# bigpon/QPNet

Measured on AMD Instinct MI355X. Metric: train steps/sec (batch-1 chunk-steps of RF+20000 samples, aggregate over GPUs), higher is better.
Workload: dtype f32; 1 GPU; config[1]: paper-size SI-QPNet (C=64,S=256,4F+4A) training step, forward+CE+backward+Adam on one chunk of 20900 samples (RF 946 + batch_length 19954), batch 1 per GPU; global_batch=1, parallelism=dp1 (utterance-sharded chunks, one flat-gradient all-reduce per step), backend=none, world_size=1, aux_1x1=frame rate (hoisted: K = 128 + one 4-deep step)

## Files before the change

### qpnet_amd/csrc/train_bwd.hip

```cpp
#include "train_common.h"
#include "train_post.h"
#include "qpn_handle.h"
#include <string.h>
#include <stdlib.h>
#include <math.h>

template <int MT>
__global__ __launch_bounds__(512) void k_post_bwd(TrainParams p, TrainBwd bw) {
    constexpr int TM = 16 * MT;
    extern __shared__ float sm[];
    const int S = p.S, Q = p.Q, LC = p.LC;
    const int ldp = tr_lda(Q > S ? Q : S), ldr = tr_lda(S);
    float* P = sm; float* R = sm + TM * ldp;
    const int b = blockIdx.y, t0 = blockIdx.x * TM;
    const int tid = threadIdx.x, lane = tid & 63, wave = tid >> 6;
    const int NTS = S / 16;
    const int npairs = (NTS + 1) / 2;
    const int np0 = wave < npairs ? wave : 0;
    const int pnt[2] = {2 * np0, (2 * np0 + 1 < NTS) ? 2 * np0 + 1 : 2 * np0};
    float my[2][MT][4], ms[2][MT][4];
    auto mask_load = [&](const float* src, float (&m)[2][MT][4]) {
#pragma unroll
        for (int j = 0; j < 2; ++j)
#pragma unroll
            for (int mt = 0; mt < MT; ++mt)
#pragma unroll
                for (int i = 0; i < 4; ++i) {
                    const int r = t0 + 16 * mt + 4 * (lane >> 4) + i;
                    m[j][mt][i] = src[((size_t)b * p.BL + r) * S + 16 * pnt[j] + (lane & 15)];
                }
    };
#define PIN8(m) asm volatile("" :: "v"(m[0][0][0]), "v"(m[0][0][1]), "v"(m[0][0][2]), "v"(m[0][0][3]), "v"(m[1][0][0]), "v"(m[1][0][1]), "v"(m[1][0][2]), "v"(m[1][0][3]))
    mask_load(p.Y0, my);
    for (int idx = tid; idx < TM * (Q / 2); idx += 512) {
        const int r = idx / (Q / 2), k = (idx - r * (Q / 2)) * 2;
        float2 v = make_float2(0.f, 0.f);
        if (t0 + r < p.BL) v = *(const float2*)(bw.dlogits + ((size_t)b * p.BL + t0 + r) * Q + k);
        *(float2*)(P + (size_t)r * ldp + k) = v;
    }
    __syncthreads();
    mask_load(p.S0, ms);
    PIN8(my);
    if (MT > 1) {
#pragma unroll
        for (int mt = 1; mt < MT; ++mt) asm volatile("" :: "v"(my[0][mt][0]), "v"(my[0][mt][1]), "v"(my[0][mt][2]), "v"(my[0][mt][3]), "v"(my[1][mt][0]), "v"(my[1][mt][1]), "v"(my[1][mt][2]), "v"(my[1][mt][3]));
    }
    for (int pb = 0; pb < npairs; pb += 8) {
        const int np = pb + wave;
        if (np < npairs) {
            const int nt0 = 2 * np, nt1 = (2 * np + 1 < NTS) ? 2 * np + 1 : 2 * np;
            f32x4 acc[MT][2];
#pragma unroll
            for (int mt = 0; mt < MT; ++mt) { acc[mt][0] = (f32x4){0, 0, 0, 0}; acc[mt][1] = (f32x4){0, 0, 0, 0}; }
            const int nts[2] = {nt0, nt1};
            wave_gemm<MT, 2>(acc, P, ldp, p.wp + p.p2t_f4, NTS, nts, Q, lane);
#pragma unroll
            for (int j = 0; j < 2; ++j) {
                if (j && nt1 == nt0) break;
// ... 360 lines not shown
#pragma unroll
            for (int i = 0; i < 4; ++i) Os[(size_t)(4 * (lane >> 4) + i) * ldo + 16 * nt + (lane & 15)] = acc[j][i];
        }
        TR_LDS_BARRIER();
#pragma unroll
        for (int i = 0; i < 4; ++i) {
            const int r = 4 * wave + i, n = n0 + r;
            const bool in = n < N1;
            const float own = Os[(size_t)r * ldo + lane] + Dx[(size_t)r * ldx + lane];
            float* da = DAout + (__umul24((unsigned)n, (unsigned)C) + lane);
            *(in ? da : dmy + lane) = own;
            const float past = Os[(size_t)r * ldo + C + lane];
            float* db = DBout + (__umul24((unsigned)tprow[i], (unsigned)C) + lane);
            db = in ? db : dmy + 128 + lane;
            if (ly.adaptive) atomicAdd(db, past);
            else *db = past;
            if constexpr (!HOIST) if (lane < Ap) {
                float* dh = DH + (__umul24((unsigned)n, (unsigned)Ap) + lane);
                atomicAdd(in ? dh : dmy + 192 + lane, Os[(size_t)r * ldo + 2 * C + lane]);
            }
        }
        if constexpr (HOIST) {
            if (lane < 16) {
                float* dp = bw.DPA + cpoff + 16 * wave + lane;
                atomicAdd(dp, dacc[0]); atomicAdd(dp + C, dacc[1]); atomicAdd(dp + 2 * C, dacc[2]); atomicAdd(dp + 3 * C, dacc[3]);
                float* ep = bw.EB + (size_t)(l * TR_EB_SLOTS + (blockIdx.x & (TR_EB_SLOTS - 1))) * 2 * C + 16 * wave + lane;
                atomicAdd(ep, eacc[0]); atomicAdd(ep + C, eacc[1]);
            }
            if (tid < 16 && n0 + tid < N1) GWl[n0 + tid] = (Gp[tid] + Gp[16 + tid]) + (Gp[32 + tid] + Gp[48 + tid]);
        }
        store_rows(t + 1 < t_last ? t + 1 : t_last, sm + ((ti + 1) & 1) * 4 * 16 * ldx);
#pragma unroll
        for (int i = 0; i < 4; ++i) tprow[i] = tpnext[i];
        if constexpr (HOIST) {
#pragma unroll
            for (int i = 0; i < 4; ++i) { cwj[i] = nwj[i]; cpa[i] = npa[i]; }
            cpoff = npoff;
        }
    }
}

struct Wg2 {
    const float* A; const float* A2; size_t A_lstride; int lda, M;
    int rowsA;
    int bmode; const float* B1; const float* B2; size_t B_lstride; int ldb, N, Nvalid;
    int rowsB;
    const float* hup; const int* tap; int C, Ap;
    const int* xc;
    int nb, nlayers;
    float* slab; int gstage;
    int row0A[TR_MAXL], row0B[TR_MAXL], R[TR_MAXL];
    int goff[TR_MAXL], gbias[TR_MAXL], tap_off[TR_MAXL], dil[TR_MAXL];
    int ldc, ncol_groups;
};

struct Wg2L {
    const float* A; const float* A2; const float* B1; const float* B2; const float* hup; const int* tap;
    int lda, ldb, M, Ng, Nvalid, rowsA, rowsB, row0A, row0B, C, Ap, dil, nb, ncol0, rend;
    unsigned uR;
};

template <int NB>
__device__ __forceinline__ void wg_taps(const Wg2L& q, int rs, int (&tp)[NB], bool b_act, int b_row0, int b_rstep) {
#pragma unroll
    for (int k = 0; k < NB; ++k) {
        const int r = b_row0 + k * b_rstep, rr = rs + r;
        int v = 0;
        if (b_act && r < 32 && rr < q.rend) {
            const unsigned b = q.nb > 1 ? (unsigned)rr / q.uR : 0u; const int i = rr - (int)(b * q.uR);
            const int nloc = q.row0B + i;
            v = q.tap ? q.tap[(size_t)b * q.rowsB + nloc] : nloc - q.dil;
        }
        tp[k] = v;
    }
}

template <int BMODE, int NA, int NB>
__device__ __forceinline__ void wg_fetch(const Wg2L& q, int rs, float4 (&ra)[NA], float4 (&ra2)[NA], float4 (&rb)[NB], float4 (&rb2)[NB], const int (&tpv)[NB],
                                         bool a_act, int a_row0, int a_rstep, int a_col, bool b_act, int b_row0, int b_rstep, int b_col) {
#pragma unroll
    for (int k = 0; k < NA; ++k) {
        const int r = a_row0 + k * a_rstep, rr = rs + r;
        float4 v = make_float4(0.f, 0.f, 0.f, 0.f), v2 = v;
        if (a_act && r < 32 && rr < q.rend && a_col < q.M) {
            const unsigned b = q.nb > 1 ? (unsigned)rr / q.uR : 0u; const int i = rr - (int)(b * q.uR);
            const size_t o = ((size_t)b * q.rowsA + q.row0A + i) * q.lda + a_col;
            v = *(const float4*)(q.A + o);
            if (q.A2) v2 = *(const float4*)(q.A2 + o);
        }
        ra[k] = v; ra2[k] = v2;
    }
#pragma unroll
    for (int k = 0; k < NB; ++k) {
        const int r = b_row0 + k * b_rstep, rr = rs + r;
        const int n = q.ncol0 + b_col;
        float4 v = make_float4(0.f, 0.f, 0.f, 0.f), v2 = make_float4(1.f, 1.f, 1.f, 1.f);
        if (b_act && r < 32 && rr < q.rend && b_col < q.Ng && n < q.Nvalid) {
            const unsigned b = q.nb > 1 ? (unsigned)rr / q.uR : 0u; const int i = rr - (int)(b * q.uR);
            const int nloc = q.row0B + i;
            const size_t row = (size_t)b * q.rowsB + nloc;
            if (BMODE <= 1) v = *(const float4*)(q.B1 + row * q.ldb + n);
            else if (BMODE == 2) { v = *(const float4*)(q.B1 + row * q.ldb + n); v2 = *(const float4*)(q.B2 + row * q.ldb + n); }
            else {
                if (n < q.C) v = *(const float4*)(q.B1 + row * q.C + n);
                else if (n < 2 * q.C) v = *(const float4*)(q.B1 + ((size_t)b * q.rowsB + tpv[k]) * q.C + (n - q.C));
                else v = *(const float4*)(q.hup + row * q.Ap + (n - 2 * q.C));
// ... 321 lines not shown
                    else v = rb[k];
                    if (BMODE == 1) { v.x = fmaxf(v.x, 0.f); v.y = fmaxf(v.y, 0.f); v.z = fmaxf(v.z, 0.f); v.w = fmaxf(v.w, 0.f); }
                    else if (BMODE == 2) { v.x *= rb2[k].x; v.y *= rb2[k].y; v.z *= rb2[k].z; v.w *= rb2[k].w; }
                    { const bool ok = (okB >> k) & 1u; v.x = ok ? v.x : 0.f; v.y = ok ? v.y : 0.f; v.z = ok ? v.z : 0.f; v.w = ok ? v.w : 0.f; }
                    *(float4*)(Bb + (size_t)r * ldB + b_col) = v;
                }
            }
        }
    };
    auto ksteps = [&](int buf, int k0, int k1) {
        const float* Ab = As + buf * BUF; const float* Bb = Bs + buf * BUF;
#pragma unroll
        for (int ks = k0; ks < k1; ++ks) {
            float bfr[NT];
#pragma unroll
            for (int nt = 0; nt < NT; ++nt) bfr[nt] = Bb[(4 * ks + g) * ldB + 16 * nt + cl];
#pragma unroll
            for (int mi = 0; mi < MPW; ++mi) {
                const float a = Ab[(4 * ks + g) * ldA + 16 * (wave + 4 * mi) + cl];
#pragma unroll
                for (int nt = 0; nt < NT; ++nt) acc[mi][nt] = __builtin_amdgcn_mfma_f32_16x16x4f32(a, bfr[nt], acc[mi][nt], 0, 0, 0);
            }
        }
    };
    for (int rs = rbeg; rs < rend; rs += RS) {
        to_lds(0);
        __syncthreads();
        if (rs + RS < rend) {
            fetch(rs + RS);
            if (BMODE == 3 && rs + 2 * RS < rend) taps(rs + 2 * RS);
        }
        ksteps(0, 0, RS / 4);
        __syncthreads();
    }
    float* out = w.slab + (size_t)ch * w.gstage;
#pragma unroll
    for (int mi = 0; mi < MPW; ++mi) {
        const int mt = wave + 4 * mi;
#pragma unroll
        for (int nt = 0; nt < NT; ++nt) {
#pragma unroll
            for (int i = 0; i < 4; ++i) {
                const int m = 16 * mt + 4 * (lane >> 4) + i, nn = 16 * nt + (lane & 15);
                out[goff + (size_t)m * w.ldc + ncol0 + nn] = acc[mi][nt][i];
            }
        }
    }
    if (gbias >= 0) {
        *(float4*)(sm + (size_t)a_row0 * Mp + a_col) = cs4;
        __syncthreads();
        if (tid < Mp) { float s = 0.f; for (int r = 0; r < ARS; ++r) s += sm[r * Mp + tid]; out[gbias + tid] = s; }
    }
}
template <int BMODE, int MPW, int NT, bool TWO_A, int MINW = 1>
__global__ __launch_bounds__(256, MINW) void k_wgrad3(Wg2 w, int nch) {
    wgrad3_body<BMODE, MPW, NT, TWO_A>(w, nch, blockIdx.x, blockIdx.y, blockIdx.z);
}

#ifndef QPN_WGRAD_MINW
#define QPN_WGRAD_MINW 2
#endif
template <int BMODE, int MPW, int NT, bool TWO_A>
static void launch_wgrad3_k(const Wg2& w, int nch, size_t lds, hipStream_t stream) {
    constexpr int MINW = (MPW == 4 && NT == 4 && !TWO_A) ? QPN_WGRAD_MINW : 1;
    if (lds > 64 * 1024) (void)hipFuncSetAttribute((const void*)k_wgrad3<BMODE, MPW, NT, TWO_A, MINW>, hipFuncAttributeMaxDynamicSharedMemorySize, (int)lds);
    hipLaunchKernelGGL((k_wgrad3<BMODE, MPW, NT, TWO_A, MINW>), dim3(nch, w.nlayers, w.ncol_groups), dim3(256), lds, stream, w, nch);
}
template <int BMODE, int MPW, int NT>
static bool wgrad3_fits(const Wg2& w) {
    const int Ng = w.N / w.ncol_groups;
    if (w.bmode != BMODE) return false;
    if (w.rowsB >= (1 << 24) || (int64_t)w.rowsB * (w.C > w.ldb ? w.C : w.ldb) >= (1ll << 32)) return false;
    if (w.M != 64 * MPW || Ng != 16 * NT || w.N % w.ncol_groups || (w.Nvalid != w.N && (w.ncol_groups != 1 || w.Nvalid % 4))) return false;
    if (BMODE == 3 && (w.ldb != w.C || w.ncol_groups != 1 || (w.C % 4) || (w.Ap % 4) || !w.tap)) return false;
    if (BMODE == 3) for (int l = 0; l < w.nlayers; ++l) if (w.tap_off[l] < 0) return false;
    return true;
}
template <int MPW, int NT> static constexpr size_t wgrad3_lds() { return (size_t)32 * (tr_ldt(64 * MPW) + tr_ldt(16 * NT)) * sizeof(float); }
template <int BMODE, int MPW, int NT>
static bool launch_wgrad3(const Wg2& w, int nch, hipStream_t stream) {
    if (!wgrad3_fits<BMODE, MPW, NT>(w)) return false;
    const size_t lds = wgrad3_lds<MPW, NT>();
    if (w.A2) launch_wgrad3_k<BMODE, MPW, NT, true>(w, nch, lds, stream);
    else launch_wgrad3_k<BMODE, MPW, NT, false>(w, nch, lds, stream);
    return true;
}
static bool wgrad3_any(const Wg2& w, int nch, bool generic, hipStream_t stream) {
    if (w.bmode == 4) return launch_wgrad3<4, 1, 8>(w, nch, stream) || launch_wgrad3<4, 1, 4>(w, nch, stream);
    if (generic) return false;
    switch (w.bmode) {
    case 3: return launch_wgrad3<3, 2, 11>(w, nch, stream) || launch_wgrad3<3, 2, 8>(w, nch, stream) || launch_wgrad3<3, 1, 7>(w, nch, stream);
    case 0: return launch_wgrad3<0, 1, 4>(w, nch, stream) || launch_wgrad3<0, 4, 4>(w, nch, stream);
    case 1: return launch_wgrad3<1, 4, 4>(w, nch, stream);
    default: return false;
    }
}

static int wgrad_col_groups(int M, int N) {
    const int nt_max = M <= 64 ? 4 : M <= 128 ? 12 : 8;
    for (int g = 1; g <= N / 16; ++g)
        if (N % g == 0 && (N / g) % 4 == 0 && (N / g + 15) / 16 <= nt_max) return g;
    return 1;
}

static bool wgrad2_any(const Wg2& w, int nch, bool generic, hipStream_t stream) {
    if (w.M > 256 && w.bmode != 4) {
        bool ok = true;
        for (int m0 = 0; m0 < w.M && ok; m0 += 256) {
            Wg2 sub = w;
            sub.A = w.A + m0; if (w.A2) sub.A2 = w.A2 + m0;
            sub.M = w.M - m0 < 256 ? w.M - m0 : 256;
            for (int l = 0; l < w.nlayers; ++l) { sub.goff[l] = w.goff[l] + m0 * w.ldc; if (w.gbias[l] >= 0) sub.gbias[l] = w.gbias[l] + m0; }
            sub.ncol_groups = wgrad_col_groups(sub.M, sub.N);
            ok = wgrad2_any(sub, nch, generic, stream);
        }
        return ok;
    }
    if (wgrad3_any(w, nch, generic, stream)) return true;
    switch (w.bmode) {
    case 4: return false;
    case 1: return wgrad2_mode<1>(w, nch, stream);
    case 2: return wgrad2_mode<2>(w, nch, stream);
    case 3: return wgrad2_mode<3>(w, nch, stream);
    default: return wgrad2_mode<0>(w, nch, stream);
    }
}

__global__ void k_reduce_grad_s(const float* __restrict__ slab, const int* __restrict__ gdst, const int* __restrict__ gdst_list, const int* __restrict__ gzero, int n_gzero,
                                int nch, int gstage, int64_t n, float* __restrict__ g, float scale, int append_scale, int s0, int s1, int skip0, int skip1, int tail,
                                const int* __restrict__ status, int flag_again) {
    int64_t i = (int64_t)blockIdx.x * blockDim.x + threadIdx.x + s0;
    if (flag_again && append_scale && i == s0) g[n + 1] = (status && *status) ? 1.f : 0.f;
    if (i < s1) {
        if (i >= skip0 && i < skip1) return;
        const int k0 = gdst[i], k1 = gdst[i + 1];
        if (k0 == k1) return;
        float a = 0.f;
        const float* sp = slab + i;
        int c = 0;
        for (; c + 8 <= nch; c += 8) {
            float v[8];
#pragma unroll
            for (int k = 0; k < 8; ++k) v[k] = sp[(size_t)(c + k) * gstage];
            a += ((v[0] + v[1]) + (v[2] + v[3])) + ((v[4] + v[5]) + (v[6] + v[7]));
        }
        for (; c < nch; ++c) a += sp[(size_t)c * gstage];
        a *= scale;
        for (int k = k0; k < k1; ++k) g[gdst_list[k]] = a;
        return;
    }
    if (!tail) return;
    const int64_t j = i - s1;
    if (j < n_gzero) g[gzero[j]] = 0.f;
    else if (append_scale && j < n_gzero + 4 && !(flag_again && j == n_gzero + 1)) g[n + (j - n_gzero)] = j == n_gzero ? scale : (j == n_gzero + 1 && status && *status) ? 1.f : 0.f;
}

__global__ __launch_bounds__(256) void k_causal_bwd(TrainParams p, TrainBwd bw, int rows_per_wg, int CB) {
    extern __shared__ float tab[];
// ... 188 lines not shown
            if (lds_c > 48 * 1024) QPN_HIP(hipFuncSetAttribute((const void*)k_causal_bwd, hipFuncAttributeMaxDynamicSharedMemorySize, (int)lds_c));
            hipLaunchKernelGGL(k_causal_bwd, dim3(nwg), dim3(256), lds_c, stream, p, bw, rpw, CB);
        }
        if (p.U > 0 && !up_done && !p.hoist) launch_up_bwd(p, bw, stream);
        if (p.hoist && ag && !up_done) launch_aux_tail(p, bw, *ag, stream);
    }
    qpn_prof_mark(PG_GRAD_TAIL, stream);
    QPN_HIP(hipGetLastError());
    return QPN_OK;
}

bool qpn_stack_bwd_fits(const TrainParams& p);
int qpn_launch_stack_bwd(const TrainParams& p, const TrainBwd& bw, const StackQ& q, const TrainKnobs& k, hipStream_t stream);
bool qpn_stack_bwd_w_fits(const TrainParams& p);
int qpn_launch_stack_bwd_w(const TrainParams& p, const TrainBwd& bw, const StackQ& q, const TrainKnobs& k, hipStream_t stream);

void qpn_launch_post_fb(const TrainParams& p, const TrainBwd& bw, hipStream_t stream) {
    constexpr int MTW = 5;
    const size_t ldsw = (size_t)16 * MTW * (tr_lda(256) + 2 * tr_lda(64)) * sizeof(float);
    (void)hipFuncSetAttribute((const void*)k_post_fb_w<MTW>, hipFuncAttributeMaxDynamicSharedMemorySize, (int)ldsw);
    hipLaunchKernelGGL((k_post_fb_w<MTW>), dim3((p.BL + 16 * MTW - 1) / (16 * MTW), p.B), dim3(512), ldsw, stream, p, bw, 1);
}

int qpn_launch_bwd(const TrainParams& p, const TrainBwd& bw, const TrainKnobs& k, const AuxGeom& ag, const StackQ* sq, hipStream_t stream, bool post_done) {
    const int C = p.C, S = p.S, Q = p.Q, L = p.L, B = p.B, N1 = p.N1, BL = p.BL;
    const TrainSlabs& sl = *bw.sl;
    const bool off32 = N1 < (1 << 24) && (int64_t)N1 * (p.LC > 2 * C ? p.LC : 2 * C) < (1ll << 32);
    const bool persist = C == 64 && (p.Ktp == 176 || p.hoist) && p.Ap <= 64 && off32 && k.persist_bwd;
    const bool stack_q = persist && k.stack_q_bwd && sq && sq->flags && p.qctl && qpn_stack_bwd_fits(p);
    const bool wr_summed = stack_q;
    const size_t nDX = (size_t)B * N1 * C;
    const size_t lds_post = (size_t)16 * (tr_lda(Q > S ? Q : S) + tr_lda(S)) * sizeof(float);
    const size_t lds_layer = (size_t)16 * (4 * tr_lda(C) + tr_lda(2 * C)) * sizeof(float);
    if (lds_post > 160 * 1024 || lds_layer > 160 * 1024) { qpn_set_error("backward tiles do not fit LDS"); return QPN_EINVAL; }
    hipStream_t side = bw.side; hipEvent_t ev_fork = bw.ev_fork, ev_join = bw.ev_join;
    const bool overlap = side && !qpn_prof_serial() && !k.serial;
    const bool post_wide = S == 256 && Q == 256 && C == 64 && (p.LC == 256 || p.LC == 512) && k.post_wide;
    const bool zero_in_post = post_wide && k.zero_in_post;
    if (post_done) { }
    else if (!zero_in_post) qpn_launch_zero_dx(p, bw, stream);
    if (post_done) { }
    else if (post_wide) {
        constexpr int MTW = 5;
        const size_t ldsw = (size_t)16 * MTW * tr_lda(256) * sizeof(float);
        QPN_HIP(hipFuncSetAttribute((const void*)k_post_bwd_w<MTW>, hipFuncAttributeMaxDynamicSharedMemorySize, (int)ldsw));
        hipLaunchKernelGGL((k_post_bwd_w<MTW>), dim3((BL + 16 * MTW - 1) / (16 * MTW), B), dim3(512), ldsw, stream, p, bw, zero_in_post ? 1 : 0);
    } else {
        if (lds_post > 48 * 1024) (void)hipFuncSetAttribute((const void*)k_post_bwd<1>, hipFuncAttributeMaxDynamicSharedMemorySize, (int)lds_post);
        hipLaunchKernelGGL((k_post_bwd<1>), dim3((BL + 15) / 16, B), dim3(512), lds_post, stream, p, bw);
    }
    qpn_prof_mark(PG_POST_BWD, stream);
    const int nch = bw.nch;
    int nch_side_ = nch;
    const bool gen = k.wgrad_generic;
    Wg2 wbase; memset(&wbase, 0, sizeof(wbase));
    wbase.slab = bw.slab; wbase.gstage = bw.gstage; wbase.nb = B; wbase.C = C; wbase.Ap = p.Ap; wbase.hup = p.HUP; wbase.tap = p.TAP; wbase.ncol_groups = 1;
    bool ok = true;
    auto launch_skip_post = [&](hipStream_t st) {
        Wg2 w = wbase;
        {
            w.nlayers = L;
            w.A = bw.DS0; w.A2 = nullptr; w.A_lstride = 0; w.lda = S; w.M = S; w.rowsA = BL;
            w.bmode = 0; w.B1 = p.TH; w.B2 = nullptr; w.B_lstride = nDX; w.ldb = C; w.N = C; w.Nvalid = C; w.rowsB = N1; w.ldc = C;
            w.ncol_groups = wgrad_col_groups(w.M, w.N);
            for (int l = 0; l < L; ++l) { w.row0A[l] = 0; w.row0B[l] = N1 - BL; w.R[l] = BL; w.goff[l] = sl.g_ws[l]; w.gbias[l] = l == 0 ? sl.g_bs : -1; w.tap_off[l] = -1; }
            ok = ok && wgrad2_any(w, nch_side_, gen, st);
            qpn_prof_mark(PG_WGRAD_SKIP, st);
        }
        {
            w.nlayers = 1; w.A_lstride = w.B_lstride = 0; w.B2 = nullptr; w.bmode = 1; w.rowsA = w.rowsB = BL;
            w.row0A[0] = w.row0B[0] = 0; w.R[0] = BL; w.tap_off[0] = -1;
            w.ncol_groups = S % 64 == 0 ? S / 64 : 1;
            w.A = bw.dlogits; w.lda = Q; w.M = Q; w.B1 = p.Y0; w.ldb = S; w.N = S; w.Nvalid = S; w.ldc = S; w.goff[0] = sl.g_p2; w.gbias[0] = sl.g_bp2;
            if (Q == S && k.post_pair) {
                w.nlayers = 2;
                w.A_lstride = (size_t)(bw.DY0 - bw.dlogits); w.B_lstride = (size_t)(p.S0 - p.Y0);
                w.row0A[1] = w.row0B[1] = 0; w.R[1] = BL; w.tap_off[1] = -1; w.goff[1] = sl.g_p1; w.gbias[1] = sl.g_bp1;
                ok = ok && wgrad2_any(w, nch_side_, gen, st);
            } else {
                ok = ok && wgrad2_any(w, nch_side_, gen, st);
                w.A = bw.DY0; w.lda = S; w.M = S; w.B1 = p.S0; w.goff[0] = sl.g_p1; w.gbias[0] = sl.g_bp1;
                ok = ok && wgrad2_any(w, nch_side_, gen, st);
            }
            qpn_prof_mark(PG_WGRAD_POST, st);
        }
    };
    auto build_w1 = [&]() {
        Wg2 w = wbase;
        w.A = bw.DZ; w.A2 = nullptr; w.A_lstride = (size_t)B * N1 * 2 * C; w.lda = 2 * C; w.M = 2 * C; w.rowsA = N1;
        w.bmode = 3; w.B1 = p.X; w.B2 = nullptr; w.B_lstride = nDX; w.ldb = C; w.N = p.Ktp; w.Nvalid = p.hoist ? 2 * C : 2 * C + p.Ap; w.rowsB = N1;
        w.nlayers = L; w.ldc = p.Ktp; w.ncol_groups = wgrad_col_groups(w.M, w.N);
        for (int l = 0; l < L; ++l) {
            const TrLayer& ly = p.layers[l];
            w.row0A[l] = w.row0B[l] = ly.s_out; w.R[l] = N1 - ly.s_out; w.goff[l] = sl.g_w1[l]; w.gbias[l] = sl.g_b1[l];
            w.tap_off[l] = ly.tap_off; w.dil[l] = ly.dilation;
        }
        return w;
    };
    auto build_wr = [&]() {
        Wg2 w = wbase;
        w.A = bw.DXA[0] + nDX; w.A2 = wr_summed ? nullptr : bw.DXB[0] + nDX; w.A_lstride = nDX; w.lda = C; w.M = C; w.rowsA = N1;
        w.bmode = 0; w.B1 = p.TH; w.B2 = nullptr; w.B_lstride = nDX; w.ldb = C; w.N = C; w.Nvalid = C; w.rowsB = N1; w.ldc = C;
        w.nlayers = L; w.ncol_groups = wgrad_col_groups(w.M, w.N);
        for (int l = 0; l < L; ++l) {
            w.row0A[l] = w.row0B[l] = p.layers[l].s_out;
            w.R[l] = l == L - 1 ? 0 : N1 - p.layers[l].s_out; w.goff[l] = sl.g_wr[l]; w.gbias[l] = sl.g_br[l]; w.tap_off[l] = -1; w.dil[l] = 0;
        }
// ... 84 lines not shown
```

### qpnet_amd/csrc/train_common.h

```cpp
#pragma once
#include "qpn_common.h"

typedef float f32x4 __attribute__((ext_vector_type(4)));

#define TR_MAXL QPN_MAX_LAYERS

__host__ __device__ static inline int tr_lda(int K) { return ((K + 29) / 32) * 32 + 2; }
__host__ __device__ static inline int tr_ldt(int N) { return ((N + 15) / 32) * 32 + 16; }

struct TrLayer {
    int adaptive, dilation;
    int s_in, s_out;
    int tap_off;
    int w1_f4, wr_f4;
    int w1t_f4, wrt_f4;
    int bias1, biasr;
};

struct TrainParams {
    int C, S, Q, A, Ap, L, U;
    int B, T, F, Td, BL, N1, N0, maxd;
    int Kt, Ktp;
    int LC;
    const float* flat;
// ... 29 lines not shown
    TrLayer layers[TR_MAXL];
};

struct TrainSlabs {
    int g_w1[TR_MAXL], g_b1[TR_MAXL], g_wr[TR_MAXL], g_br[TR_MAXL], g_ws[TR_MAXL], g_bs;
    int g_p1, g_bp1, g_p2, g_bp2;
    int g_early0, g_early1;
    int g_cw, g_cb;
};

struct TrainBwd {
    const float* dlogits; float* gflat;
    float* DXA[2]; float* DXB[2];
    float* DZ;
    float* DS0; float* DY0;
    float* DGS;
    float* DHUP;
    float* DPA;
    float* GW;
    float* EB;
    float* slab;
    const int* gdst; const int* gdst_list;
    const int* gzero; int n_gzero;
    int nch, gstage;
    int64_t n_params;
    const struct TrainSlabs* sl;
    float gscale;
    int append_scale;
    const int* status;
    hipStream_t side; hipEvent_t ev_fork, ev_join, ev_mid;
    hipEvent_t ev_early; int* early_recorded;
};


struct AuxGeom { int auxS[TR_MAXL], auxT[TR_MAXL], bias1[TR_MAXL], s_out[TR_MAXL]; };
struct AuxArgs {
    const float* flat; const float* h; float* PA; float* bp; const float* DPA; const float* EB; const float* GW; float* gflat;
    float gscale; int C, A, L, B, F, U, N1, nfr, ffirst; int64_t up_w, up_b;
    AuxGeom g;
};
static inline AuxArgs tr_aux_args(const TrainParams& p, const TrainBwd* bw, const AuxGeom& ag) {
    AuxArgs a; a.flat = p.flat; a.h = p.h; a.PA = p.PA; a.bp = p.bp; a.DPA = bw ? bw->DPA : nullptr; a.EB = bw ? bw->EB : nullptr; a.GW = bw ? bw->GW : nullptr;
    a.gflat = bw ? bw->gflat : nullptr; a.gscale = bw ? bw->gscale : 1.f;
    a.C = p.C; a.A = p.A; a.L = p.L; a.B = p.B; a.F = p.F; a.U = p.U; a.N1 = p.N1; a.nfr = p.nfr; a.ffirst = p.ffirst; a.up_w = p.up_w; a.up_b = p.up_b; a.g = ag;
    return a;
}
struct TrainKnobs {
    bool serial;
    bool stack_q_fwd, stack_q_bwd;
    int stack_wgs, stack_wgs_bwd;
    bool persist_fwd, persist_bwd;
    bool wgrad_generic;
    int wgrad_chunks, wgrad_chunks_side;
    bool post_fuse;
    bool up_side, reduce_early, wr_side;
    bool post_pair, zero_in_post, post_wide;
    bool xcd_swizzle;
    bool ce_separate;
    bool event_fence;
    bool aux_hoist;
    int stack_wave_fwd; bool stack_wave_bwd;
    int stack_waves;
    bool test_stack_gives_up;
};
void qpn_train_knobs_parse(TrainKnobs& k);

#define TR_QHEAD_STRIDE 1056
#define TR_QHDR_WORDS 17920
struct StackQ {
    unsigned* flags;
    unsigned* head;
    unsigned* stats;
    unsigned* abort;
    const int4* tab;
    unsigned epoch;
    unsigned epoch_pub;
    unsigned spin_limit;
    int total, nq;
};

__host__ __device__ __forceinline__ int tr_pa_off(const TrainParams& p, int l, int b, int n0) {
    const int q = p.F * p.U - p.N1 + n0;
    return ((l * p.B + b) * (p.nfr + 1) + (q / p.U - p.ffirst)) * 2 * p.C;
}

__device__ __forceinline__ void tr_queue_entry_fwd(const TrainParams& p, int pos, int4& a, int4& b) {
    const bool valid = pos < p.qtotal;
    const int ps = valid ? pos : 0;
    int l = 0;
    for (int k = 1; k < p.L; ++k) l += ps >= p.qP[k] ? 1 : 0;
    const int r = ps - p.qP[l], T = p.qT[l];
    const int bi = r / T, t = r - bi * T;
    const TrLayer ly = p.layers[l];
    const int n0 = ly.s_out + 16 * t;
    int first = 0, n = 0;
    if (valid && l > 0) {
        const int reach = ly.s_out - ly.s_in, s_prev = p.layers[l - 1].s_out;
        int lo = n0 - reach; if (lo < s_prev) lo = s_prev;
        int hi = n0 + 15; if (hi > p.N1 - 1) hi = p.N1 - 1;
        const int t_lo = (lo - s_prev) >> 4, t_hi = (hi - s_prev) >> 4;
        first = p.qP[l - 1] + bi * p.qT[l - 1] + t_lo; n = t_hi - t_lo + 1;
    }
    a = make_int4(n0, l | (bi << 8) | (l == p.L - 1 ? 1 << 24 : 0) | (valid ? 1 << 25 : 0), first, n);
    b = make_int4((l * p.B + bi) * p.N1, ly.tap_off + bi * p.N1, p.hoist ? tr_pa_off(p, l, bi, n0) : bi * p.N1, 0);
}

// ... 239 lines not shown
```

### qpnet_amd/csrc/train_host.hip

```cpp
#include "train_common.h"
#include "qpn_handle.h"
#include <algorithm>
#include <string.h>

int qpn_launch_fwd(const TrainParams& p, const TrainKnobs& k, const AuxGeom& ag, const StackQ* sq, hipStream_t stream, const TrainBwd* fuse_post_bwd);
void qpn_stack_fill(TrainParams& p);
int qpn_launch_ce(const float* logits, const int64_t* tgt, int64_t tgt_stride, int B, int BL, int Q, float* dlogits, double* loss, int* status, bool loss_cleared, hipStream_t stream);
int qpn_launch_bwd(const TrainParams& p, const TrainBwd& bw, const TrainKnobs& k, const AuxGeom& ag, const StackQ* sq, hipStream_t stream, bool post_done);
int qpn_launch_fwd_gemm(const TrainParams& p, const TrainGemm& w, hipStream_t stream);
int qpn_launch_bwd_gemm(const TrainParams& p, const TrainBwd& bw, const TrainGemm& w, hipStream_t stream);
int qpn_launch_adam(float* w, const float* g, float* m, float* v, int64_t n, int step, float lr, float b1, float b2, float eps, float wd, const float* den, int* status,
                    int* h_status, double* h_loss, const double* d_loss, hipStream_t stream);


struct TrainState {
    std::vector<int> h_wmap;
    std::vector<int> h_bstart, h_blist;
    std::vector<int> h_gsrc;
    int* d_wmap; float* d_wp; int* d_bstart; int* d_blist; float* d_bp; int n_bias;
    int* d_gdst; int* d_gdst_list; int* d_gzero; int n_gzero;
    bool hoist;
    TrainParams tp;
    TrainBwd bw;
    TrainSlabs slabs;
    TrainKnobs knobs;
    AuxGeom ag;
    float* d_ws; size_t ws_cap;
    int* d_tap; size_t tap_cap;
    int* d_status; double* d_loss;
    hipStream_t last_stream;
    int* h_status_pinned; hipEvent_t ev_status[2]; bool status_pending[2]; int status_newest;
    double* h_loss_pinned; hipEvent_t ev_loss[2]; bool loss_pending[2]; int loss_newest;
    bool fwd_valid;
    bool loss_clear;
    bool use_gemm;
    int* d_ctmap; float* d_ct;
    std::vector<int> h_gmap; int* d_gmap; float* d_gwp;
    TrainGemm gm;
    int64_t generation;
    hipStream_t side; hipEvent_t ev_fork, ev_join, ev_mid;
    hipEvent_t ev_early; int early_recorded; int64_t early_first;
    int64_t bwd_generation;
    const float* post_bwd_dlogits;
    bool post_bwd_done;
    bool stack_disabled;
    unsigned* d_sq; size_t sq_pos_cap, sq_per_dir;
    StackQ sqf, sqb;
};

static int env_int(const char* name, int dflt) { const char* e = getenv(name); return (e && *e) ? atoi(e) : dflt; }
void qpn_train_knobs_parse(TrainKnobs& k) {
    k.serial = env_int("QPN_TRAIN_SERIAL", 0) != 0;
    k.stack_q_fwd = env_int("QPN_STACK_QUEUE", 1) != 0;
    k.stack_q_bwd = k.stack_q_fwd && env_int("QPN_STACK_QUEUE_BWD", 1) != 0;
    k.stack_wgs = env_int("QPN_STACK_WGS", 0); if (k.stack_wgs < 0 || k.stack_wgs > 4096) k.stack_wgs = 0;
    k.stack_wgs_bwd = env_int("QPN_STACK_WGS_BWD", 0); if (k.stack_wgs_bwd < 0 || k.stack_wgs_bwd > 4096) k.stack_wgs_bwd = 0;
    k.persist_fwd = env_int("QPN_LAYER_PERSIST", 1) != 0;
    k.persist_bwd = env_int("QPN_LAYER_BWD_PERSIST", 1) != 0;
    k.wgrad_generic = getenv("QPN_WGRAD_GENERIC") != nullptr;
    k.wgrad_chunks = env_int("QPN_WGRAD_CHUNKS", 0); if (k.wgrad_chunks < 1 || k.wgrad_chunks > 512) k.wgrad_chunks = 0;
    k.wgrad_chunks_side = env_int("QPN_WGRAD_CHUNKS_SIDE", 0); if (k.wgrad_chunks_side < 1 || k.wgrad_chunks_side > 512) k.wgrad_chunks_side = 0;
    k.up_side = env_int("QPN_UP_SIDE", 1) != 0;
    k.reduce_early = env_int("QPN_REDUCE_EARLY", 1) != 0;
    k.wr_side = env_int("QPN_WR_SIDE", 1) != 0;
    k.post_fuse = env_int("QPN_POST_FUSE", 1) != 0;
    k.post_pair = env_int("QPN_POST_WGRAD_PAIR", 1) != 0;
    k.zero_in_post = env_int("QPN_ZERO_IN_POST", 1) != 0;
    k.post_wide = env_int("QPN_POST_WIDE", 1) != 0;
    k.xcd_swizzle = getenv("QPN_NO_XCD_SWIZZLE") == nullptr;
    k.ce_separate = getenv("QPN_CE_SEPARATE") != nullptr;
    k.event_fence = env_int("QPN_EVENT_FENCE", 0) == 1;
    k.aux_hoist = env_int("QPN_AUX_HOIST", 1) != 0;
    k.stack_wave_fwd = env_int("QPN_STACK_WAVE_FWD", 0);
    k.stack_wave_bwd = env_int("QPN_STACK_WAVE_BWD", 0) != 0;
    k.stack_waves = 4;
    k.test_stack_gives_up = false;
#ifdef QPN_TESTING
    k.test_stack_gives_up = env_int("QPN_TEST_STACK_GIVES_UP", 0) == 1;
#endif
}

int qpn_num_cus() {
    static int cached[64] = {0};
    int dev = 0;
    if (hipGetDevice(&dev) != hipSuccess || dev < 0 || dev >= 64) return 256;
    if (!cached[dev]) { int n = 0; if (hipDeviceGetAttribute(&n, hipDeviceAttributeMultiprocessorCount, dev) != hipSuccess || n < 1) n = 256; cached[dev] = n; }
    return cached[dev];
}

struct Prof { bool on = false; bool overlapped = false; std::vector<hipEvent_t> ev; std::vector<int> grp; std::vector<hipStream_t> st; size_t used = 0; };
static thread_local Prof g_prof;
bool qpn_prof_active() { return g_prof.on; }
bool qpn_prof_serial() { return g_prof.on && !g_prof.overlapped; }
void qpn_prof_mark(int group, hipStream_t stream) {
    Prof& P = g_prof;
    if (!P.on) return;
    if (P.used == P.ev.size()) { hipEvent_t e; if (hipEventCreate(&e) != hipSuccess) return; P.ev.push_back(e); P.grp.push_back(0); P.st.push_back(nullptr); }
    P.grp[P.used] = group; P.st[P.used] = stream;
    (void)hipEventRecord(P.ev[P.used++], stream);
}
extern "C" int qpn_train_profile_begin(qpn_handle* h, void* stream) {
    (void)h; g_prof.on = true; g_prof.overlapped = false; g_prof.used = 0;
    qpn_prof_mark(-1, (hipStream_t)stream);
    return QPN_OK;
}
extern "C" int qpn_train_profile_begin_overlapped(qpn_handle* h, void* stream) {
    (void)h; g_prof.on = true; g_prof.overlapped = true; g_prof.used = 0;
    qpn_prof_mark(-1, (hipStream_t)stream);
    return QPN_OK;
}
extern "C" int qpn_train_profile_mark(qpn_handle* h, int group, void* stream) {
    (void)h; qpn_prof_mark(group, (hipStream_t)stream); return QPN_OK;
}
extern "C" int qpn_train_profile_end(qpn_handle* h, float* h_ms, int n, void* stream) {
// ... 727 lines not shown
```

Before: 1475 steps/s.

## Add multi-buffered direct-to-LDS DMA pipeline for weight-gradient GEMM kernels

Adds a new weight-gradient body that loads A and B row tiles straight into shared memory with global_load_lds_dwordx4, using a 3- or 4-stage ring buffer with vmcnt-based waits. This lets loads overlap MFMA compute and skips the register round-trip. It is enabled by default for the bmode 3 (2x8) and bmode 0/1 (4x4) configurations and can be turned off with environment knobs. In exchange it uses more LDS, which can lower occupancy, and it relies on inline asm and m0 handling that could be fragile.

```diff
diff --git a/qpnet_amd/csrc/train_bwd.hip b/qpnet_amd/csrc/train_bwd.hip
--- a/qpnet_amd/csrc/train_bwd.hip
+++ b/qpnet_amd/csrc/train_bwd.hip
@@ -4,6 +4,7 @@
 #include <string.h>
 #include <stdlib.h>
 #include <math.h>
+#include <type_traits>
 
 template <int MT>
 __global__ __launch_bounds__(512) void k_post_bwd(TrainParams p, TrainBwd bw) {
@@ -470,6 +471,7 @@
     int row0A[TR_MAXL], row0B[TR_MAXL], R[TR_MAXL];
     int goff[TR_MAXL], gbias[TR_MAXL], tap_off[TR_MAXL], dil[TR_MAXL];
     int ldc, ncol_groups;
+    int dma;
 };
 
 struct Wg2L {
@@ -897,14 +899,221 @@
         if (tid < Mp) { float s = 0.f; for (int r = 0; r < ARS; ++r) s += sm[r * Mp + tid]; out[gbias + tid] = s; }
     }
 }
+template <int SR, int Mp, int Np> struct WgDmaGeom {
+    static constexpr int A4 = Mp / 4, RPIA = 64 / A4, B4 = Np / 4, RPIB = 64 / B4;
+    static constexpr int ldA = RPIA == 1 ? Mp + 16 : Mp, ldB = Np;
+    static constexpr int AIS = RPIA == 1 ? ldA : 256;
+    static constexpr int JA = SR / RPIA / 4, JB = SR / RPIB / 4;
+    static constexpr int STAGE = SR * (ldA + ldB);
+    static_assert((Mp == 256 || Mp == 128) && (Np == 128 || Np == 64) && JA >= 1 && JB >= 1, "rows of 64, 128 or 256 floats");
+};
+static constexpr int wg_vmcnt(int n) { return 0x0F70 | (n & 15) | ((n >> 4) << 14); }
+__device__ __forceinline__ void wg_glds16(const float* src, float* dst) {
+    const unsigned lds = __builtin_amdgcn_readfirstlane((unsigned)(size_t)(__attribute__((address_space(3))) void*)dst);
+    unsigned keep;
+    asm volatile("s_mov_b32 %0, m0\n\ts_mov_b32 m0, %2\n\ts_nop 0\n\tglobal_load_lds_dwordx4 %1, off\n\ts_mov_b32 m0, %0" : "=&s"(keep) : "v"(src), "s"(lds) : "memory");
+}
+
+template <int BMODE, int MPW, int NT, int NBUF, int SR>
+__device__ __forceinline__ void wgrad3_dma_body(const Wg2& w, const int nch, const int ch, const int y, const int zg) {
+    extern __shared__ float sm[];
+    constexpr int RS = 32, Mp = 64 * MPW, Np = 16 * NT;
+    using G = WgDmaGeom<SR, Mp, Np>;
+    constexpr int A4 = G::A4, RPIA = G::RPIA, B4 = G::B4, RPIB = G::RPIB, ldA = G::ldA, ldB = G::ldB, AIS = G::AIS, JA = G::JA, JB = G::JB, STAGE = G::STAGE;
+    constexpr int J = JA + JB;
+    constexpr int ARS = 256 / A4, NAS = SR / ARS;
+    static_assert(NBUF >= 2 && NBUF <= 4 && (SR == 16 || SR == 32) && (NBUF - 2) * J < 64, "ring depth");
+    const int tid = threadIdx.x, lane = tid & 63, wave = __builtin_amdgcn_readfirstlane(tid >> 6);
+    const int Rl = w.R[y];
+    const int64_t total = (int64_t)Rl * w.nb;
+    const int64_t per = ((total + nch - 1) / nch + RS - 1) / RS * RS;
+    const int rbeg = (int)(per * ch), rend = (int)(per * ch + per < total ? per * ch + per : total);
+    const float* A = w.A + (size_t)y * w.A_lstride;
+    const float* B1 = w.B1 + (size_t)y * w.B_lstride;
+    const int* tap = BMODE == 3 ? w.tap + w.tap_off[y] : nullptr;
+    const int row0A = w.row0A[y], row0B = w.row0B[y], ncol0 = zg * Np;
+    const unsigned uR = (unsigned)(Rl > 0 ? Rl : 1);
+    const bool multi = w.nb > 1;
+    const int gbias = zg == 0 ? w.gbias[y] : -1, goff = w.goff[y];
+    int* tapL = (int*)(sm + NBUF * STAGE);
+    const int ar0 = wave * (JA * RPIA) + lane / A4, agc = lane % A4;
+    const int asc = RPIA > 1 ? (agc ^ ((ar0 & 1) << 2)) : agc;
+    const int br0 = wave * (JB * RPIB) + lane / B4, bgc = lane % B4;
+    const int bsc = bgc ^ ((br0 & 1) << 2);
+    const bool use_tap = BMODE == 3 && 4 * bsc >= w.C;
+    const int bcol = BMODE == 3 ? (use_tap ? 4 * bsc - w.C : 4 * bsc) : ncol0 + 4 * bsc;
+    const int bstride = BMODE == 3 ? w.C : w.ldb;
+    const unsigned a_voff = (unsigned)ar0 * (unsigned)w.lda + 4u * (unsigned)asc, a_jstep = (unsigned)RPIA * (unsigned)w.lda;
+    const unsigned b_voff = (unsigned)br0 * (unsigned)w.ldb + (unsigned)bcol, b_jstep = (unsigned)RPIB * (unsigned)w.ldb;
+
+    f32x4 acc[MPW][NT];
+#pragma unroll
+    for (int a = 0; a < MPW; ++a)
+#pragma unroll
+        for (int b = 0; b < NT; ++b) acc[a][b] = (f32x4){0, 0, 0, 0};
+    float4 cs4 = make_float4(0.f, 0.f, 0.f, 0.f);
+    auto rowsplit = [&](int rr, int& b, int& i) { if (multi) { b = (int)((unsigned)rr / uR); i = rr - b * (int)uR; } else { b = 0; i = rr; } };
+
+    if (BMODE == 3) {
+        for (int k = tid; k < rend - rbeg; k += 256) {
+            int b, i; rowsplit(rbeg + k, b, i);
+            tapL[k] = tap[(size_t)b * w.rowsB + row0B + i];
+        }
+        __syncthreads();
+    }
+    auto issue = [&](int rs, int buf) {
+        const float* pa[JA]; const float* pb[JB];
+        int b0, i0; rowsplit(rs, b0, i0);
+        if (rs + SR <= rend && i0 + SR <= (int)uR) {
+            const float* Ast = A + ((size_t)b0 * w.rowsA + row0A + i0) * w.lda;
+#pragma unroll
+            for (int j = 0; j < JA; ++j) pa[j] = Ast + (a_voff + j * a_jstep);
+            if (BMODE == 3) {
+                const float* Bst = B1 + (size_t)b0 * w.rowsB * w.C + bcol;
+#pragma unroll
+                for (int j = 0; j < JB; ++j) {
+                    const int r = br0 + j * RPIB;
+                    const unsigned row = use_tap ? (unsigned)tapL[rs - rbeg + r] : (unsigned)(row0B + i0 + r);
+                    pb[j] = Bst + __umul24(row, (unsigned)w.C);
+                }
+            } else {
+                const float* Bst = B1 + ((size_t)b0 * w.rowsB + row0B + i0) * w.ldb;
+#pragma unroll
+                for (int j = 0; j < JB; ++j) pb[j] = Bst + (b_voff + j * b_jstep);
+            }
+        } else {
+#pragma unroll
+            for (int j = 0; j < JA; ++j) {
+                int rr = rs + ar0 + j * RPIA; rr = rr < rend ? rr : rend - 1;
+                int b, i; rowsplit(rr, b, i);
+                pa[j] = A + (((size_t)b * w.rowsA + row0A + i) * w.lda + 4 * asc);
+            }
+#pragma unroll
+            for (int j = 0; j < JB; ++j) {
+                int rr = rs + br0 + j * RPIB; rr = rr < rend ? rr : rend - 1;
+                int b, i; rowsplit(rr, b, i);
+                const size_t row = (size_t)b * w.rowsB + (use_tap ? tapL[rr - rbeg] : row0B + i);
+                pb[j] = B1 + (row * bstride + bcol);
+            }
+        }
+        float* Ab = sm + buf * STAGE + wave * (JA * AIS); float* Bb = sm + buf * STAGE + SR * ldA + wave * (JB * 256);
+#pragma unroll
+        for (int j = 0; j < JA; ++j) wg_glds16(pa[j], Ab + j * AIS);
+#pragma unroll
+        for (int j = 0; j < JB; ++j) wg_glds16(pb[j], Bb + j * 256);
+    };
+    const int g = lane >> 4, cl = lane & 15;
+    const int a_frag = g * ldA + cl + 16 * (RPIA > 1 ? (wave ^ (g & 1)) : wave);
+    const int b_frag_e = g * ldB + cl + 16 * (g & 1), b_frag_o = g * ldB + cl - 16 * (g & 1);
+    auto ksteps = [&](int buf) {
+        const float* Ab = sm + buf * STAGE + a_frag; const float* Be = sm + buf * STAGE + SR * ldA + b_frag_e; const float* Bo = sm + buf * STAGE + SR * ldA + b_frag_o;
+#pragma unroll
+        for (int ks = 0; ks < SR / 4; ++ks) {
+            float bfr[NT];
+#pragma unroll
+            for (int nt = 0; nt < NT; ++nt) {
+                bfr[nt] = ((nt & 1) ? Bo : Be)[4 * ks * ldB + 16 * nt];
+                if (BMODE == 1) bfr[nt] = fmaxf(bfr[nt], 0.f);
+            }
+#pragma unroll
+            for (int mi = 0; mi < MPW; ++mi) {
+                const float a = Ab[4 * ks * ldA + 64 * mi];
+#pragma unroll
+                for (int nt = 0; nt < NT; ++nt) acc[mi][nt] = __builtin_amdgcn_mfma_f32_16x16x4f32(a, bfr[nt], acc[mi][nt], 0, 0, 0);
+            }
+        }
+    };
+    const int a_row0 = tid / A4, a_col = (tid % A4) * 4;
+    const int cs_off = a_row0 * ldA + (RPIA > 1 ? (a_col ^ ((a_row0 & 1) << 4)) : a_col);
+    const int nst = (rend - rbeg + SR - 1) / SR;
+    for (int s = 0; s < NBUF - 1 && s < nst; ++s) issue(rbeg + s * SR, s);
+    int buf = 0;
+    auto stage = [&](int s, auto ahead, auto more) {
+        __builtin_amdgcn_s_waitcnt(wg_vmcnt(decltype(ahead)::value * J));
+        asm volatile("s_waitcnt lgkmcnt(0)" ::: "memory");
+        __builtin_amdgcn_s_barrier();
+        const int rs = rbeg + s * SR;
+        if constexpr (decltype(more)::value) if (s + NBUF - 1 < nst) issue(rs + (NBUF - 1) * SR, buf == 0 ? NBUF - 1 : buf - 1);
+        if (rs + SR > rend) {
+            float* Ab = sm + buf * STAGE; float* Bb = Ab + SR * ldA;
+            const int nv = rend - rs;
+            for (int i = nv * ldA + 4 * tid; i < SR * ldA; i += 1024) *(float4*)(Ab + i) = make_float4(0.f, 0.f, 0.f, 0.f);
+            for (int i = nv * ldB + 4 * tid; i < SR * ldB; i += 1024) *(float4*)(Bb + i) = make_float4(0.f, 0.f, 0.f, 0.f);
+            asm volatile("s_waitcnt lgkmcnt(0)" ::: "memory");
+            __builtin_amdgcn_s_barrier();
+        }
+        if (gbias >= 0) {
+            const float* Ab = sm + buf * STAGE + cs_off;
+#pragma unroll
+            for (int k = 0; k < NAS; ++k) { const float4 v = *(const float4*)(Ab + k * ARS * ldA); cs4.x += v.x; cs4.y += v.y; cs4.z += v.z; cs4.w += v.w; }
+        }
+        ksteps(buf);
+        buf = buf + 1 == NBUF ? 0 : buf + 1;
+    };
+    int s = 0;
+    for (; s + (NBUF - 2) < nst; ++s) stage(s, std::integral_constant<int, NBUF - 2>(), std::true_type());
+    if constexpr (NBUF >= 4) if (s + 1 < nst) { stage(s, std::integral_constant<int, 1>(), std::false_type()); ++s; }
+    if constexpr (NBUF >= 3) if (s < nst) { stage(s, std::integral_constant<int, 0>(), std::false_type()); ++s; }
+    asm volatile("s_waitcnt lgkmcnt(0)" ::: "memory");
+    __builtin_amdgcn_s_barrier();
+    float* out = w.slab + (size_t)ch * w.gstage;
+#pragma unroll
+    for (int mi = 0; mi < MPW; ++mi) {
+        const int mt = wave + 4 * mi;
+#pragma unroll
+        for (int nt = 0; nt < NT; ++nt) {
+#pragma unroll
+            for (int i = 0; i < 4; ++i) {
+                const int m = 16 * mt + 4 * (lane >> 4) + i, nn = 16 * nt + (lane & 15);
+                out[goff + (size_t)m * w.ldc + ncol0 + nn] = acc[mi][nt][i];
+            }
+        }
+    }
+    if (gbias >= 0) {
+        *(float4*)(sm + (size_t)a_row0 * Mp + a_col) = cs4;
+        __syncthreads();
+        if (tid < Mp) { float s = 0.f; for (int r = 0; r < ARS; ++r) s += sm[r * Mp + tid]; out[gbias + tid] = s; }
+    }
+}
+template <int BMODE, int MPW, int NT, bool TWO_A> static constexpr bool wg_has_dma = !TWO_A && ((BMODE == 3 && MPW == 2 && NT == 8) || ((BMODE == 0 || BMODE == 1) && MPW == 4 && NT == 4));
+
 template <int BMODE, int MPW, int NT, bool TWO_A, int MINW = 1>
 __global__ __launch_bounds__(256, MINW) void k_wgrad3(Wg2 w, int nch) {
+    if constexpr (wg_has_dma<BMODE, MPW, NT, TWO_A>) {
+        switch (w.dma) {
+        case 316: wgrad3_dma_body<BMODE, MPW, NT, 3, 16>(w, nch, blockIdx.x, blockIdx.y, blockIdx.z); return;
+        case 416: wgrad3_dma_body<BMODE, MPW, NT, 4, 16>(w, nch, blockIdx.x, blockIdx.y, blockIdx.z); return;
+        default: break;
+        }
+    }
     wgrad3_body<BMODE, MPW, NT, TWO_A>(w, nch, blockIdx.x, blockIdx.y, blockIdx.z);
 }
 
 #ifndef QPN_WGRAD_MINW
 #define QPN_WGRAD_MINW 2
 #endif
+struct WgOpt { bool generic; int dma, dma_side; };
+template <int BMODE, int MPW, int NT>
+static size_t wgrad3_dma_lds(const Wg2& w, int nch, int ring) {
+    constexpr int Mp = 64 * MPW, Np = 16 * NT;
+    if (w.nb < 1 || nch < 1 || w.Nvalid != w.N) return 0;
+    if (BMODE == 3 && (2 * w.C != Np || w.C % 32)) return 0;
+    size_t stage;
+    switch (ring) {
+    case 316: case 416: stage = WgDmaGeom<16, Mp, Np>::STAGE; break;
+    default: return 0;
+    }
+    size_t words = (size_t)(ring / 100) * stage;
+    if (BMODE == 3) {
+        int64_t per_max = 0;
+        for (int l = 0; l < w.nlayers; ++l) {
+            const int64_t total = (int64_t)w.R[l] * w.nb, per = ((total + nch - 1) / nch + 31) / 32 * 32;
+            if (per > per_max) per_max = per;
+        }
+        words += (size_t)per_max;
+    }
+    return words * sizeof(float) <= (size_t)160 * 1024 ? words * sizeof(float) : 0;
+}
 template <int BMODE, int MPW, int NT, bool TWO_A>
 static void launch_wgrad3_k(const Wg2& w, int nch, size_t lds, hipStream_t stream) {
     constexpr int MINW = (MPW == 4 && NT == 4 && !TWO_A) ? QPN_WGRAD_MINW : 1;
@@ -922,21 +1131,30 @@
     return true;
 }
 template <int MPW, int NT> static constexpr size_t wgrad3_lds() { return (size_t)32 * (tr_ldt(64 * MPW) + tr_ldt(16 * NT)) * sizeof(float); }
+#define WG_DMA_RING_W1 316
+#define WG_DMA_RING_SIDE 316
 template <int BMODE, int MPW, int NT>
-static bool launch_wgrad3(const Wg2& w, int nch, hipStream_t stream) {
+static bool launch_wgrad3(const Wg2& w, int nch, hipStream_t stream, const WgOpt& opt) {
     if (!wgrad3_fits<BMODE, MPW, NT>(w)) return false;
-    const size_t lds = wgrad3_lds<MPW, NT>();
-    if (w.A2) launch_wgrad3_k<BMODE, MPW, NT, true>(w, nch, lds, stream);
-    else launch_wgrad3_k<BMODE, MPW, NT, false>(w, nch, lds, stream);
+    size_t lds = wgrad3_lds<MPW, NT>();
+    if (w.A2) { launch_wgrad3_k<BMODE, MPW, NT, true>(w, nch, lds, stream); return true; }
+    Wg2 wd = w; wd.dma = 0;
+    if constexpr (wg_has_dma<BMODE, MPW, NT, false>) {
+        int ring = BMODE == 3 ? opt.dma : opt.dma_side;
+        if (ring == 1) ring = BMODE == 3 ? WG_DMA_RING_W1 : WG_DMA_RING_SIDE;
+        const size_t l = ring ? wgrad3_dma_lds<BMODE, MPW, NT>(w, nch, ring) : 0;
+        if (l) { wd.dma = ring; lds = l; }
+    }
+    launch_wgrad3_k<BMODE, MPW, NT, false>(wd, nch, lds, stream);
     return true;
 }
-static bool wgrad3_any(const Wg2& w, int nch, bool generic, hipStream_t stream) {
-    if (w.bmode == 4) return launch_wgrad3<4, 1, 8>(w, nch, stream) || launch_wgrad3<4, 1, 4>(w, nch, stream);
-    if (generic) return false;
+static bool wgrad3_any(const Wg2& w, int nch, const WgOpt& opt, hipStream_t stream) {
+    if (w.bmode == 4) return launch_wgrad3<4, 1, 8>(w, nch, stream, opt) || launch_wgrad3<4, 1, 4>(w, nch, stream, opt);
+    if (opt.generic) return false;
     switch (w.bmode) {
-    case 3: return launch_wgrad3<3, 2, 11>(w, nch, stream) || launch_wgrad3<3, 2, 8>(w, nch, stream) || launch_wgrad3<3, 1, 7>(w, nch, stream);
-    case 0: return launch_wgrad3<0, 1, 4>(w, nch, stream) || launch_wgrad3<0, 4, 4>(w, nch, stream);
-    case 1: return launch_wgrad3<1, 4, 4>(w, nch, stream);
+    case 3: return launch_wgrad3<3, 2, 11>(w, nch, stream, opt) || launch_wgrad3<3, 2, 8>(w, nch, stream, opt) || launch_wgrad3<3, 1, 7>(w, nch, stream, opt);
+    case 0: return launch_wgrad3<0, 1, 4>(w, nch, stream, opt) || launch_wgrad3<0, 4, 4>(w, nch, stream, opt);
+    case 1: return launch_wgrad3<1, 4, 4>(w, nch, stream, opt);
     default: return false;
     }
 }
@@ -948,7 +1166,7 @@
     return 1;
 }
 
-static bool wgrad2_any(const Wg2& w, int nch, bool generic, hipStream_t stream) {
+static bool wgrad2_any(const Wg2& w, int nch, const WgOpt& generic, hipStream_t stream) {
     if (w.M > 256 && w.bmode != 4) {
         bool ok = true;
         for (int m0 = 0; m0 < w.M && ok; m0 += 256) {
@@ -1243,7 +1461,7 @@
     qpn_prof_mark(PG_POST_BWD, stream);
     const int nch = bw.nch;
     int nch_side_ = nch;
-    const bool gen = k.wgrad_generic;
+    const WgOpt gen{k.wgrad_generic, k.wgrad_dma, k.wgrad_dma_side};
     Wg2 wbase; memset(&wbase, 0, sizeof(wbase));
     wbase.slab = bw.slab; wbase.gstage = bw.gstage; wbase.nb = B; wbase.C = C; wbase.Ap = p.Ap; wbase.hup = p.HUP; wbase.tap = p.TAP; wbase.ncol_groups = 1;
     bool ok = true;
diff --git a/qpnet_amd/csrc/train_common.h b/qpnet_amd/csrc/train_common.h
--- a/qpnet_amd/csrc/train_common.h
+++ b/qpnet_amd/csrc/train_common.h
@@ -105,6 +105,7 @@
     bool persist_fwd, persist_bwd;
     bool wgrad_generic;
     int wgrad_chunks, wgrad_chunks_side;
+    int wgrad_dma, wgrad_dma_side;
     bool post_fuse;
     bool up_side, reduce_early, wr_side;
     bool post_pair, zero_in_post, post_wide;
diff --git a/qpnet_amd/csrc/train_host.hip b/qpnet_amd/csrc/train_host.hip
--- a/qpnet_amd/csrc/train_host.hip
+++ b/qpnet_amd/csrc/train_host.hip
@@ -60,6 +60,8 @@
     k.wgrad_generic = getenv("QPN_WGRAD_GENERIC") != nullptr;
     k.wgrad_chunks = env_int("QPN_WGRAD_CHUNKS", 0); if (k.wgrad_chunks < 1 || k.wgrad_chunks > 512) k.wgrad_chunks = 0;
     k.wgrad_chunks_side = env_int("QPN_WGRAD_CHUNKS_SIDE", 0); if (k.wgrad_chunks_side < 1 || k.wgrad_chunks_side > 512) k.wgrad_chunks_side = 0;
+    k.wgrad_dma = env_int("QPN_WGRAD_DMA", 1); if (k.wgrad_dma < 0) k.wgrad_dma = 0;
+    k.wgrad_dma_side = env_int("QPN_WGRAD_DMA_SIDE", k.wgrad_dma); if (k.wgrad_dma_side < 0) k.wgrad_dma_side = 0;
     k.up_side = env_int("QPN_UP_SIDE", 1) != 0;
     k.reduce_early = env_int("QPN_REDUCE_EARLY", 1) != 0;
     k.wr_side = env_int("QPN_WR_SIDE", 1) != 0;
```

After: 1493 steps/s (median of 6 runs). 1.01x the previous value.
